# Tetramputechture/nclone

Measured on AMD Instinct MI355X. Metric: env-steps/sec (whole node) at N parallel envs, higher is better.
Workload: dtype f64

## Files before the change

include/npp_amd.h:

```cpp
#ifndef NPP_AMD_H
#define NPP_AMD_H

#include <stdint.h>

#ifdef __cplusplus
extern "C" {
#endif

typedef struct npp_handle_s *npp_handle;

enum {
    NPP_OK = 0,
    NPP_ERR_INVALID = 1,
    NPP_ERR_HIP = 2,
    NPP_ERR_UNSUPPORTED = 3,
    NPP_ERR_STATE = 4
};

enum {
    NPP_FLAG_AUTORESET = 1u << 0,
    NPP_FLAG_ALLOW_UNSUPPORTED = 1u << 1,
    NPP_FLAG_FRAME_CENTERED = 1u << 2,
    NPP_FLAG_FAST_RESET = 1u << 3
};
// ... 47 lines not shown
int npp_set_truncation_limit(npp_handle h, const int32_t *limits, int32_t all);
int npp_set_dynamic_truncation(npp_handle h, int enable);
int npp_level_truncation_limit(const double *map, int64_t n, int32_t *limit, int32_t *surface_area);

int npp_step(npp_handle h, const uint8_t *d_actions, int frame_skip, const npp_step_out *out);

int npp_step_many(npp_handle h, const uint8_t *d_actions, int n_steps, int frame_skip, const npp_step_out *out);

int npp_tick(npp_handle h, const uint8_t *d_inputs, int n_ticks);

int npp_observe(npp_handle h, const npp_step_out *out);

int npp_render_player_frame(npp_handle h, uint8_t *d_out);
int npp_set_entity_pos(npp_handle h, int env, int kind, double x, double y);

int npp_switch_states(npp_handle h, float *d_out);

int npp_reachability(npp_handle h, float *d_features, float *d_mine_sdf, int32_t *d_status);
int npp_reachability_ex(npp_handle h, float *d_features, float *d_mine_sdf, int32_t *d_status, float *d_switch_states);

int npp_set_minimal_observation(npp_handle h, int enable);
int npp_minimal_encode_host(const uint32_t *state_a, const double *planes, int count, float *out);
int npp_minimal_observation(npp_handle h, float *d_out , int32_t *d_status );

int npp_render_frame(npp_handle h, int env0, int count, uint8_t *d_out);

int npp_render_global_view(npp_handle h, uint8_t *d_out);

int npp_dump_state(npp_handle h, int env0, int count, double *f64_out, int32_t *i32_out);

int npp_dump_entities(npp_handle h, int env, int32_t *out, int max, int *n_out);

int npp_dump_level_segments(npp_handle h, int level, int16_t *out, int max_rows, int *n_out);

int npp_compile_level_segments(const double *map, int64_t n, int16_t *out, int max_rows, int *n_out,
                               uint32_t *unsupported_mask);
int npp_compile_level_entities(const double *map, int64_t n, double *out, int max_rows, int *n_out);

int npp_set_step_variant(npp_handle h, int variant);
int npp_get_step_variant(npp_handle h, int *variant, int *tuned);

int npp_set_obs_overlap(npp_handle h, int percent);
int npp_set_obs_overlap_parts(npp_handle h, const int *cuts, int n_cuts);
int npp_join(npp_handle h);

int npp_reach_compile(const double *map, int64_t n, int32_t *info, uint8_t *base_in, uint8_t *base_adj, uint8_t *phys, uint8_t *in,
// ... 43 lines not shown
```

nclone_amd/_native.py:

```python
import ctypes as C
import os

_HERE = os.path.dirname(os.path.abspath(__file__))
LIB_PATH = os.environ.get("NPP_AMD_LIB") or os.path.join(_HERE, "libnpp_amd.so")

NPP_OK = 0
NPP_ERR_INVALID, NPP_ERR_HIP, NPP_ERR_UNSUPPORTED, NPP_ERR_STATE = 1, 2, 3, 4
FLAG_AUTORESET = 1
FLAG_ALLOW_UNSUPPORTED = 2
FLAG_FRAME_CENTERED = 4
FLAG_FAST_RESET = 8
F_WON, F_DEAD, F_SWITCH, F_TRUNCATED, F_CAUSE_MINE, F_CAUSE_IMPACT = 1, 2, 4, 8, 16, 32
GAME_STATE_DIM = 41
MINIMAL_OBS_DIM = 40
DUMP_F64 = 12
DUMP_I32 = 32

EXPORTS = [
    "npp_create", "npp_destroy", "npp_last_error", "npp_set_stream", "npp_sync", "npp_load_levels",
    "npp_assign_levels", "npp_reset", "npp_set_truncation_limit", "npp_step", "npp_tick", "npp_observe",
    "npp_render_player_frame", "npp_dump_state", "npp_dump_entities", "npp_dump_level_segments",
    "npp_compile_level_segments", "npp_compile_level_entities", "npp_set_step_variant", "npp_get_step_variant", "npp_num_envs", "npp_num_levels",
    "npp_set_launch_geometry", "npp_get_launch_geometry", "npp_snapshot", "npp_restore", "npp_entity_checksum", "npp_compile_level_zoo", "npp_render_global_view", "npp_switch_states", "npp_set_entity_pos", "npp_step_many", "npp_render_frame", "npp_plan_zoo_block", "npp_reset_ex",
    "npp_reachability", "npp_reachability_ex", "npp_reach_compile", "npp_reach_features_host", "npp_reach_compile_miss", "npp_reach_rollout_host", "npp_set_dynamic_truncation", "npp_level_truncation_limit",
    "npp_set_obs_overlap", "npp_set_obs_overlap_parts", "npp_join",
    "npp_set_frame_stack", "npp_frame_stack_render", "npp_frame_stack_push", "npp_frame_stack_view",
    "npp_set_level_pool", "npp_draw_levels", "npp_get_env_levels", "npp_env_level_view", "npp_level_pool_draw_host",
    "npp_graph_observation", "npp_graph_compile",
    "npp_set_minimal_observation", "npp_minimal_observation", "npp_minimal_encode_host",
]


class StepOut(C.Structure):
    _fields_ = [
        ("d_game_state", C.c_void_p),
        ("d_action_mask", C.c_void_p),
        ("d_entity_pos", C.c_void_p),
        ("d_flags", C.c_void_p),
        ("d_reward", C.c_void_p),
        ("d_frames", C.c_void_p),
        ("d_terminal_state", C.c_void_p),
        ("d_spatial_context", C.c_void_p),
        ("d_positions", C.c_void_p),
        ("d_work", C.c_void_p),
    ]


class NativeLibraryMissing(RuntimeError):
    pass


_lib = None
# ... 55 lines not shown
    L.npp_reach_features_host.argtypes = [C.POINTER(C.c_double), C.c_int64, C.c_void_p, C.c_void_p, C.c_int, C.c_void_p, C.c_void_p,
                                          C.c_void_p]
    L.npp_reach_compile_miss.argtypes = [C.POINTER(C.c_double), C.c_int64] + [C.c_void_p] * 4
    L.npp_reach_rollout_host.argtypes = [C.POINTER(C.c_double), C.c_int64, C.c_void_p, C.c_void_p, C.c_void_p, C.c_int, C.c_void_p, C.c_void_p, C.c_void_p]
    L.npp_set_dynamic_truncation.argtypes = [H, C.c_int]
    L.npp_level_truncation_limit.argtypes = [C.POINTER(C.c_double), C.c_int64, C.POINTER(C.c_int32), C.POINTER(C.c_int32)]
    L.npp_snapshot.argtypes = [H]
    L.npp_restore.argtypes = [H, C.POINTER(C.c_uint8)]
    L.npp_set_frame_stack.argtypes = [H, C.c_int, C.c_int, C.c_int]
    L.npp_frame_stack_render.argtypes = [H]
    L.npp_frame_stack_push.argtypes = [H, C.c_void_p, C.c_void_p, C.c_void_p, C.c_int, C.c_int, C.c_void_p]
    L.npp_frame_stack_view.argtypes = [H, C.c_int, C.POINTER(C.c_void_p), C.POINTER(C.c_int64), C.POINTER(C.c_int64)]
    L.npp_set_level_pool.argtypes = [H, C.POINTER(C.c_double), C.c_int, C.c_uint64]
    L.npp_draw_levels.argtypes = [H, C.POINTER(C.c_uint8)]
    L.npp_get_env_levels.argtypes = [H, C.POINTER(C.c_int32)]
    L.npp_env_level_view.argtypes = [H, C.POINTER(C.c_void_p)]
    L.npp_graph_observation.argtypes = [H, C.c_void_p, C.c_void_p, C.c_void_p, C.c_void_p, C.c_int]
    L.npp_graph_compile.argtypes = [C.POINTER(C.c_double), C.c_int64, C.c_void_p, C.c_void_p, C.c_void_p]
    L.npp_level_pool_draw_host.argtypes = [C.POINTER(C.c_double), C.c_int, C.c_uint64, C.POINTER(C.c_int32), C.POINTER(C.c_uint32), C.c_int,
                                           C.POINTER(C.c_int32)]
    L.npp_set_minimal_observation.argtypes = [H, C.c_int]
    L.npp_minimal_observation.argtypes = [H, C.c_void_p, C.c_void_p]
    L.npp_minimal_encode_host.argtypes = [C.c_void_p, C.c_void_p, C.c_int, C.c_void_p]
    L.npp_num_envs.argtypes = [H]
    L.npp_num_levels.argtypes = [H]
    for name in EXPORTS:
        if name != "npp_last_error":
            getattr(L, name).restype = C.c_int
    _lib = L
    return L


class NppError(RuntimeError):
    def __init__(self, code, msg):
        super().__init__("npp error %d: %s" % (code, msg))
        self.code = code


def check(handle, code):
    if code != NPP_OK:
        msg = lib().npp_last_error(handle)
        raise NppError(code, msg.decode() if msg else "?")
```

nclone_amd/build_native.py:

```python
import os
import subprocess
import sys

HERE = os.path.dirname(os.path.abspath(__file__))
CSRC = os.path.join(HERE, "csrc")
OUT = os.path.join(HERE, "libnpp_amd.so")
SOURCES = ["npp_kernels.hip", "npp_render.hip", "npp_stack.hip", "npp_pool.hip", "npp_reach_kernel.hip", "npp_graph.hip", "npp_capi.cpp", "npp_level.cpp", "npp_reach.cpp",
           "npp_graph.cpp", "npp_host.cpp"]
HEADERS = ["npp_internal.hpp", "npp_level.hpp", "npp_zoo.hpp", "npp_reach.hpp", "npp_reach_build.hpp", "npp_reach_features.hpp",
           "npp_host.hpp", "npp_zoo_layout.hpp", "npp_pool.hpp", "npp_graph.hpp", "npp_minimal.hpp",
           "npp_reach_tables.inc", os.path.join("..", "..", "include", "npp_amd.h")]


def needs_build():
    if not os.path.isfile(OUT):
        return True
    t = os.path.getmtime(OUT)
    for f in SOURCES + HEADERS:
        if os.path.getmtime(os.path.join(CSRC, f)) > t:
            return True
    return False


def build(force=False, verbose=False, out=None, extra_flags=()):
    if out is None and not force and not needs_build():
        return OUT
    hipcc = os.environ.get("HIPCC", "/opt/rocm/bin/hipcc")
    objdir = os.path.join(HERE, "_obj") if out is None else out + "_obj"
    out = OUT if out is None else out
    os.makedirs(objdir, exist_ok=True)
    flags = ["--offload-arch=gfx950", "-O3", "-std=c++17", "-fPIC", "-ffp-contract=off", "-fno-fast-math", "-Wall",
             "-Wno-unused-function", "-Wno-unused-value", "-Wno-unused-result", "-I", os.path.join(HERE, "..", "include")]
    flags += list(extra_flags)
# ... 43 lines not shown
```

nclone_amd/csrc/npp_host.cpp:

```cpp
#include "npp_host.hpp"

#include <cstring>

#include "../../include/npp_amd.h"
#include "npp_minimal.hpp"
#include "npp_pool.hpp"
#include "npp_reach_build.hpp"

using namespace npp;

namespace npp {
std::string &host_error() {
    static thread_local std::string e;
    return e;
}
}

namespace {
int fail(std::nullptr_t, int code, const std::string &msg) {
    host_error() = msg;
    return code;
}
}

extern "C" {

int npp_minimal_encode_host(const uint32_t *state_a, const double *planes, int count, float *out) {
    if (count < 0 || (count > 0 && (!state_a || !planes || !out))) return fail(nullptr, NPP_ERR_INVALID, "npp_minimal_encode_host: bad arguments");
    for (int i = 0; i < count; i++)
        minobs_encode_state(state_a[i], planes[4 * i], planes[4 * i + 1], planes[4 * i + 2], planes[4 * i + 3], out + (size_t)i * MINOBS_DIM);
    return NPP_OK;
}

int npp_level_pool_draw_host(const double *weights, int n_levels, uint64_t seed, const int32_t *envs, const uint32_t *counts, int count,
                             int32_t *out) {
    if (count < 0 || (count > 0 && (!envs || !counts || !out))) return fail(nullptr, NPP_ERR_INVALID, "npp_level_pool_draw_host: bad arguments");
    std::vector<double> cdf;
    int last = 0;
    std::string err;
    if (!pool_cdf(weights, n_levels, n_levels, cdf, last, err)) return fail(nullptr, NPP_ERR_INVALID, err);
    for (int i = 0; i < count; i++) out[i] = pool_pick(cdf.data(), n_levels, last, seed, (uint32_t)envs[i], counts[i]);
    return NPP_OK;
}

int npp_compile_level_segments(const double *map, int64_t n, int16_t *out, int max_rows, int *n_out, uint32_t *unsupported_mask) {
    if (!map || !out || !n_out) return fail(nullptr, NPP_ERR_INVALID, "npp_compile_level_segments: bad arguments");
    CompiledLevel L;
    std::string err;
    if (!compile_level(map, n, L, err)) return fail(nullptr, NPP_ERR_INVALID, "npp_compile_level_segments: " + err);
    int r = dump_segments(L, out, max_rows);
    if (r < 0) return fail(nullptr, NPP_ERR_INVALID, "npp_compile_level_segments: buffer too small");
    *n_out = r;
    if (unsupported_mask) *unsupported_mask = L.unsupported_mask;
// ... 85 lines not shown
```

nclone_amd/csrc/npp_kernels.hip:

```cpp
#include <hip/hip_runtime.h>

#include <algorithm>
#include <vector>

#include <type_traits>

#include "npp_internal.hpp"
#include "npp_level.hpp"

#pragma clang fp contract(off)

namespace npp {
namespace {

constexpr double NINJA_RADIUS = 10.0;
constexpr double GRAVITY_FALL = 0.06666666666666665;
constexpr double GRAVITY_JUMP = 0.01111111111111111;
constexpr double GROUND_ACCEL = 0.06666666666666665;
constexpr double AIR_ACCEL = 0.04444444444444444;
constexpr double DRAG_REGULAR = 0.9933221725495059;
constexpr double DRAG_SLOW = 0.8617738760127536;
constexpr double FRICTION_GROUND = 0.9459290248857720;
constexpr double FRICTION_GROUND_SLOW = 0.8617738760127536;
constexpr double FRICTION_WALL = 0.9113380468927672;
constexpr double MAX_HOR_SPEED = 3.333;
constexpr int MAX_JUMP_DURATION = 45;
constexpr double MAX_SURVIVABLE_IMPACT = 6.0;
constexpr double TWO_THIRDS = 2.0 / 3;
constexpr double LEN45 = 0x1.0f876ccdf6cd9p+5;
// ... 461 lines not shown
    0x1.db00000000000p+9 ,
    0x1.e100000000000p+9 ,
    0x1.e700000000000p+9 ,
    0x1.ed00000000000p+9 ,
    0x1.f300000000000p+9 ,
    0x1.f900000000000p+9 ,
    0x1.fefffffffffffp+9 ,
    0x1.0280000000000p+10 ,
    0x1.0580000000000p+10
};

template <int K> struct Cand {
    double rx0, ry0, rx1, ry1;
    bool ok;
    uint32_t s[K];
    double x1[K], y1[K], x2[K], y2[K];
    double wx[K], wy[K], l2[K], rl2[K];
    double ox[K], oy[K];
    double bx0[K], by0[K], bx1[K], by1[K];
    double tx0[K], tx1[K], ty0[K], ty1[K];
};

template <int G, int K>
DEV void cand_gather(const Lv &lv, int r, double qx0, double qy0, double qx1, double qy1, Cand<K> &c) {
    const int c0x = cell_coord(qx0, 43), c1x = cell_coord(qx1, 43), c0y = cell_coord(qy0, 24), c1y = cell_coord(qy1, 24);
    c.rx0 = 24.0 * c0x; c.rx1 = 24.0 * (c1x + 1); c.ry0 = 24.0 * c0y; c.ry1 = 24.0 * (c1y + 1);
    const int ncol = c1x - c0x + 1;
    int a0 = lv.seg_start[c0x * 25 + c0y], n0 = lv.seg_start[c0x * 25 + c1y + 1] - a0;
    int a1 = 0, n1 = 0, a2 = 0, n2 = 0;
    if (ncol > 1) { a1 = lv.seg_start[(c0x + 1) * 25 + c0y]; n1 = lv.seg_start[(c0x + 1) * 25 + c1y + 1] - a1; }
    if (ncol > 2) { a2 = lv.seg_start[(c0x + 2) * 25 + c0y]; n2 = lv.seg_start[(c0x + 2) * 25 + c1y + 1] - a2; }
    const int total = n0 + n1 + n2;
    c.ok = ncol <= 3 && total <= G * K;
#pragma unroll
    for (int k = 0; k < K; k++) {
        int f = k * G + r;
        c.s[k] = 0;
        c.x1[k] = 0; c.y1[k] = 0; c.x2[k] = 0; c.y2[k] = 0; c.wx[k] = 0; c.wy[k] = 0; c.l2[k] = 1; c.rl2[k] = 1;
        c.ox[k] = 0; c.oy[k] = 0; c.bx0[k] = 0; c.by0[k] = 0; c.bx1[k] = 0; c.by1[k] = 0;
        c.tx0[k] = 0; c.tx1[k] = 0; c.ty0[k] = 0; c.ty1[k] = 0;
        if (c.ok && f < total) {
            int xc = c0x, i = a0 + f;
            if (f >= n0) { xc += 1; i = a1 + (f - n0); }
            if (f >= n0 + n1) { xc += 1; i = a2 + (f - n0 - n1); }
            uint32_t s = lv.segs[i];
            int yc = s >> 11;
            uint32_t cb = lv.bounds[xc * 25 + yc];
            c.s[k] = s | ((uint32_t)xc << 16) | 0x80000000u;
// ... 629 lines not shown
    if (in_jump_buffer || new_jump_check) {
        if (n.walled || in_wall_buffer) { wall_jump(n); return; }
        if (in_floor_buffer) { floor_jump(n); return; }
        if (lp && in_lp_buffer && new_jump_check) {
            n.fbuf = -1; n.wbuf = -1; n.jbuf = -1; n.lbuf = -1;
            double boost_scalar = 2 * dabs(lp[0]) + 2;
            if (boost_scalar == 2) boost_scalar = 1.7;
            n.vx += lp[0] * boost_scalar * TWO_THIRDS;
            n.vy += lp[1] * boost_scalar * TWO_THIRDS;
            return;
        }
    }
    if (!n.walled) {
        if (n.state == 5) n.state = 4;
    } else if (n.state == 5) {
        if (n.hor * n.wn <= 0) n.vy *= FRICTION_WALL;
        else n.state = 4;
    } else if (n.vy > 0 && n.hor * n.wn < 0) {
        if (n.state == 3) n.gjump = 0;
        n.state = 5;
    }
}

template <int G, bool ZOO, int V>
DEV void sim_tick(const Lv &lv, const Zoo &z, int r, Nj &n, EntBits eb, int hor, int jump, int n_ent STAMP_ARG) {
    constexpr int K = VariantK<G, ZOO, V>::value;
    STAMP_INIT;
    asm volatile("" : "+v"(hor), "+v"(jump));
    n.frame += 1;
    n.hor = hor;
    n.jump = jump;
    const bool zoo = ZOO && z.on;
    if (zoo) zoo_entities_tick<G>(lv, z, r, n, eb, n_ent);
    else think_mines(lv, n, eb);
    STAMP(2);
    if (n.state == 9) return;
    if (n.state != 6) {
        double drag = n.dslow ? DRAG_SLOW : DRAG_REGULAR;
        n.vx *= drag;
        n.vy *= drag;
        n.vy += n.gjump ? GRAVITY_JUMP : GRAVITY_FALL;
        double xold = n.x, yold = n.y;
        n.x += n.vx;
        n.y += n.vy;
        n.vxo = n.vx; n.vyo = n.vy;
        n.fcount = 0; n.ccount = 0;
        double fnsx = 0, fnsy = 0, cnsx = 0, cnsy = 0;
        ZTick zt;
        zt.xcr = 0; zt.ycr = 0; zt.clen = 0; zt.crushable = 0; zt.gcx = 0; zt.gcy = 0; zt.phys_near = false;
        if (zoo) zoo_pre_collision<G>(lv, z, r, n, zt);
        if constexpr (!ZOO) {
            if (r == 0) {
                double *sp = lv.spill;
                sp[0] = n.vxo; sp[1] = n.vyo; sp[2] = n.fnx; sp[3] = n.fny; sp[4] = n.cnx; sp[5] = n.cny;
                int *ip = reinterpret_cast<int *>(sp + 8);
                ip[0] = n.fair; ip[1] = n.scf; ip[2] = n.frame; ip[3] = n.gold; ip[4] = n.doors; ip[5] = n.fastord;
            }
            asm volatile("" ::: "memory");
        }
        Cand<K> cd;
        {
            const double pad = NINJA_RADIUS + 2.2;
            cand_gather<G, K>(lv, r, (xold < n.x ? xold : n.x) - pad, (yold < n.y ? yold : n.y) - pad,
                              (xold > n.x ? xold : n.x) + pad, (yold > n.y ? yold : n.y) + pad, cd);
        }
        STAMP(3);
        Crush cr{0, 0, 0};
        for (int k = 0; k < 4; k++) {
            const double xb = n.x, yb = n.y;
            if (zoo && zt.phys_near) {
                cr.xcr = zt.xcr; cr.ycr = zt.ycr; cr.clen = zt.clen;
                collide_vs_objects<G>(lv, z, r, n, zt, xold, yold, fnsx, fnsy, cnsx, cnsy);
                cr.xcr = zt.xcr; cr.ycr = zt.ycr; cr.clen = zt.clen;
            }
            const int applied = collide_vs_tiles<G, K, ZOO>(lv, r, n, cd, xold, yold, fnsx, fnsy, cnsx, cnsy, cr STAMP_PASS);
            n.work += applied;
            zt.xcr = cr.xcr; zt.ycr = cr.ycr; zt.clen = cr.clen;
            if (!(zoo && zt.phys_near) && applied == 0 && n.x == xb && n.y == yb) break;
        }
        STAMP(4);
        if constexpr (!ZOO) {
            asm volatile("" ::: "memory");
            const double *sp = lv.spill;
            n.vxo = sp[0]; n.vyo = sp[1]; n.fnx = sp[2]; n.fny = sp[3]; n.cnx = sp[4]; n.cny = sp[5];
            const int *ip = reinterpret_cast<const int *>(sp + 8);
            n.fair = ip[0]; n.scf = ip[1]; n.frame = ip[2]; n.gold = ip[3]; n.doors = ip[4]; n.fastord = ip[5];
        }
        post_collision<G, K, ZOO>(lv, z, r, n, cd, eb, fnsx, fnsy, cnsx, cnsy, xold, yold, zt);
        STAMP(5);
    }
    ninja_think(n, zoo ? z.blk : nullptr);
    STAMP(6);
}

DEV void write_game_state(const Nj &n, int limit, float *o ) {
    double vmag = dsqrt(sq(n.vx) + sq(n.vy));
    o[0] = (float)(pymin(vmag / (MAX_HOR_SPEED * 2), 1.0) * 2 - 1);
    bool mv = vmag > 1e-6;
    o[1] = (float)(mv ? n.vx / vmag : 0.0);
    o[2] = (float)(mv ? n.vy / vmag : 0.0);
    o[3] = (n.state <= 2) ? 1.f : -1.f;
    o[4] = (n.state == 3 || n.state == 4) ? 1.f : -1.f;
    o[5] = (n.state == 5) ? 1.f : -1.f;
    o[6] = (n.state >= 6 && n.state <= 9) ? 1.f : -1.f;
    o[7] = n.airborn ? 1.f : -1.f;
    o[8] = (float)n.hor;
    o[9] = n.jump ? 1.f : -1.f;
    o[10] = (float)(((n.jbuf > 0 ? n.jbuf : 0) / 5.0) * 2 - 1);
    o[11] = (float)(((n.fbuf > 0 ? n.fbuf : 0) / 5.0) * 2 - 1);
    o[12] = (float)(((n.wbuf > 0 ? n.wbuf : 0) / 5.0) * 2 - 1);
    o[13] = (float)((n.fcount < 1 ? n.fcount : 1) * 2 - 1);
    o[14] = -1.f;
    o[15] = (float)((n.ccount < 1 ? n.ccount : 1) * 2 - 1);
    o[16] = (float)(dsqrt(sq(n.fnx) + sq(n.fny)) * 2 - 1);
    o[17] = 0.f;
    o[18] = (float)n.fny;
    double g = n.gjump ? GRAVITY_JUMP : GRAVITY_FALL;
    o[19] = (float)((g - GRAVITY_JUMP) / (GRAVITY_FALL - GRAVITY_JUMP) * 2 - 1);
    o[20] = n.walled ? 1.f : -1.f;
    o[21] = (float)n.fnx;
    o[22] = (float)n.cnx;
    o[23] = (float)n.cny;
    double drag = n.dslow ? DRAG_SLOW : DRAG_REGULAR;
    o[24] = (float)((drag - DRAG_SLOW) / (DRAG_REGULAR - DRAG_SLOW) * 2 - 1);
    o[25] = (float)((FRICTION_GROUND - FRICTION_GROUND_SLOW) / (FRICTION_GROUND - FRICTION_GROUND_SLOW) * 2 - 1);
    o[26] = (float)pymax(-1.0, pymin(1.0, (n.vx - n.vxo) / MAX_HOR_SPEED));
    o[27] = (float)pymax(-1.0, pymin(1.0, (n.vy - n.vyo) / MAX_HOR_SPEED));
    o[28] = (float)(pymin(vmag / (MAX_HOR_SPEED * 1.5), 1.0) * 2 - 1);
    o[29] = (float)(pymin(n.fair / 60.0, 1.0) * 2 - 1);
    o[30] = (float)(pymin(n.jdur / (double)MAX_JUMP_DURATION, 1.0) * 2 - 1);
    o[31] = (float)(pymin(n.scf / 30.0, 1.0) * 2 - 1);
    double ke = 0.5 * (sq(n.vx) + sq(n.vy));
    o[32] = (float)(pymin(ke / sq(MAX_HOR_SPEED), 1.0) * 2 - 1);
    o[33] = (float)((n.y / 600.0) * 2 - 1);
    double fm = dsqrt(sq(g) + sq(!n.airborn ? GROUND_ACCEL : AIR_ACCEL));
    o[34] = (float)(pymin(fm / 0.1, 1.0) * 2 - 1);
    double pke = 0.5 * (sq(n.vxo) + sq(n.vyo));
    o[35] = (float)pymax(-1.0, pymin(1.0, (ke - pke) / pymax(ke + 0.01, 0.01)));
    o[36] = (float)(pymin(n.fcount / 5.0, 1.0) * 2 - 1);
    o[37] = -1.f;
    o[38] = (float)(atan2(n.fny, n.fnx) / 3.141592653589793);
    o[39] = n.walled ? (float)n.wn : 0.f;
    o[40] = (float)(limit <= 0 ? 1.0 : pymax(0.0, (double)(limit - n.frame) / (double)limit));
}

DEV uint32_t action_mask_bits(const Nj &n) {
    uint32_t mask = 0x3f;
    bool has_active_buffer = (-1 < n.jbuf && n.jbuf < 5) || (-1 < n.fbuf && n.fbuf < 5) || (-1 < n.wbuf && n.wbuf < 5) ||
                             (-1 < n.lbuf && n.lbuf < 4);
    if (n.airborn && n.state != 3 && n.jump != 0 && !has_active_buffer) mask &= ~(8u | 16u | 32u);
    if (n.walled) {
        bool masks_dir = !n.airborn || n.state == 5 || !(n.vy >= 0);
        if (masks_dir) { if (n.wn > 0) mask &= ~2u; else if (n.wn < 0) mask &= ~4u; }
    }
    if (!mask) mask = 1;
    return mask;
}

template <int G>
DEV void write_spatial_context(const KernelArgs &a, const LevelHdr &H, Nj &n, EntBits eb, int env, int r, bool valid) {
    if (!valid) return;
    float *out = a.out.spatial_context + (size_t)env * 112;
    float *cache = a.sc_cache + (size_t)env * 48;
    const uint8_t *tiles = a.blob + H.off_tiles;
    const int col = floor12(n.x) >> 1, row = floor12(n.y) >> 1;
    for (int k = r; k < 64; k += G) {
        int rr = row - 4 + (k >> 3), cc = col - 4 + (k & 7);
// ... 98 lines not shown
    spawn_state(lv, n);
    n.fastord = episode;
    if (fast) {
        n.fastord |= 1;
        lv.perm = reinterpret_cast<const uint16_t *>(a.blob + H.off_ent_perm);
        const uint32_t *keep = reinterpret_cast<const uint32_t *>(a.blob + H.off_keep_words);
        for (int w = 0; w < nw; w++) {
            const uint32_t k = keep[w];
            eb.w[w * eb.stride] = (eb.w[w * eb.stride] & k) | (lv.init_words[w] & ~k);
        }
        if constexpr (ZOO) {
            z.ent_ord = reinterpret_cast<const uint16_t *>(a.blob + H.off_ent_rank);
            if (z.on) zoo_fast_reset_block(z, r, G);
        }
    } else {
        lv.perm = reinterpret_cast<const uint16_t *>(a.blob + H.off_ent_ident);
        for (int w = 0; w < nw; w++) eb.w[w * eb.stride] = lv.init_words[w];
        if constexpr (ZOO) {
            z.ent_ord = z.ent_seq;
            if (z.on) zoo_init_block(z, r, G, false);
        }
    }
}

template <int G, bool LDS_LEVEL, bool ZOO, bool MANY, int V>
DEV void run(const KernelArgs &a, unsigned char *smem) {
    constexpr int EPW = WAVE / G;
    const int tid = threadIdx.x;
    const int wave = tid >> 6;
    const int lane = tid & 63;
    const int r = lane & (G - 1);
    const int epb = EPW * (blockDim.x >> 6);
    const int eib = wave * EPW + lane / G;
    const int blk = a.wg_order ? (int)a.wg_order[blockIdx.x + a.wg_first] : (int)blockIdx.x + a.wg_first;
    const unsigned long long wg_t0 = a.wg_cost ? __builtin_amdgcn_s_memtime() : 0ull;
    const int env0 = blk * epb;
    const int env = env0 + eib;
    const bool in_range = env < a.n;
    const bool valid = in_range && (!a.obs_mask || a.obs_mask[env] != 0);
    if (a.obs_mask && !__syncthreads_or(valid)) return;
    const int e = in_range ? env : a.n - 1;
    const int n_valid = (a.n - env0) < epb ? (a.n - env0) : epb;

    uint32_t *ew = reinterpret_cast<uint32_t *>(smem + (LDS_LEVEL ? a.lds_hot_cap : 0u));
    uint32_t *stage = ew + (size_t)a.n_words_max * epb;
    EntBits eb;
// ... 67 lines not shown
#ifdef NPP_STAMPS
    Stamps st;
    for (int i = 0; i < N_STAMP; i++) st.acc[i] = 0;
#endif
    STAMP_INIT;
    Nj n;
    load_state(a, e, n);
    lv.perm = reinterpret_cast<const uint16_t *>(a.blob + ((n.fastord & 1) ? H.off_ent_perm : H.off_ent_ident));
    if constexpr (ZOO) {
        if (n.fastord & 1) z.ent_ord = reinterpret_cast<const uint16_t *>(a.blob + H.off_ent_rank);
    }
    const int nw = (int)lv.n_words;
    if (r == 0)
        for (int w = 0; w < nw; w++) eb.w[w * eb.stride] = a.ent_bits[(size_t)w * a.n + e];
    __syncthreads();

    STAMP(0);
    uint32_t flags = 0;
    int executed = 0;
    float reward = 0.f;
    bool done = false;
    const bool stepping = a.mode == 0 && a.n_ticks > 0;
    const bool writer = valid && r == 0;
    const int n_steps = MANY ? (a.n_steps > 1 ? a.n_steps : 1) : 1;
#pragma nounroll
    for (int sidx = 0; sidx < n_steps; sidx++) {
        flags = 0; executed = 0; reward = 0.f;
        n.work = 0;
        const bool had_switch = lv.obs_switch >= 0 && ent_get(eb, lv.obs_switch) == 0;
        {
            const bool gym = a.mode == 0;
            const int act = (gym && a.n_ticks > 0) ? a.inputs[(size_t)sidx * a.n + e] : 0;
            int hor = (act == 1 || act == 4) ? -1 : ((act == 2 || act == 5) ? 1 : 0);
            int jump = act >= 3 ? 1 : 0;
            bool live = valid && !(gym && (n.state == 8 || n.state == 6 || n.state == 7));
            for (int t = 0; t < a.n_ticks; t++) {
                if (!gym) {
                    const int b = a.inputs[(size_t)t * a.n + e];
                    const int l = (b >> 2) & 1, rr = (b >> 1) & 1;
                    hor = (l && rr) ? 0 : (l ? -1 : (rr ? 1 : 0));
                    jump = b & 1;
                }
                if (live) {
                    sim_tick<G, ZOO, V>(lv, z, r, n, eb, hor, jump, (int)H.n_ent STAMP_PASS);
                    executed++;
                    if (gym && (n.state == 8 || n.state == 6 || n.state == 7)) live = false;
                }
                if (!__any(live)) break;
            }
        }

        STAMP(1);
        const bool sw_now = lv.obs_switch >= 0 ? ent_get(eb, lv.obs_switch) == 0 : true;
        if (n.state == 8) flags |= 1u;
        if (n.state == 6 || n.state == 7) flags |= 2u;
        if (sw_now) flags |= 4u;
        if (n.cause == 1) flags |= 16u;
        if (n.cause == 2) flags |= 32u;
        done = (flags & 3u) != 0;
        if (stepping && !done && n.frame >= a.trunc_limit[e]) { flags |= 8u; done = true; }
        if (flags & 1u) reward += 20.f;
        if (flags & 2u) reward -= 3.f;
        if (sw_now && !had_switch && lv.obs_switch >= 0) reward += 10.f;

        if (writer) {
            const size_t o = (size_t)sidx * a.n + env;
            if (a.out.flags) a.out.flags[o] = (uint8_t)flags;
            if (a.out.reward) a.out.reward[o] = reward;
            if (a.out.frames) a.out.frames[o] = (uint16_t)executed;
            if (a.out.work) a.out.work[o] = (uint16_t)(n.work > 0xffff ? 0xffff : n.work);
        }
        if (MANY && sidx + 1 < n_steps && a.autoreset && stepping && done)
            episode_reset<ZOO>(a, H, lv, z, n, eb, nw, r, G);
    }

    const bool do_reset = a.autoreset && stepping && done;
#pragma nounroll
    for (int pass = (a.out.terminal_state ? 0 : 1); pass < 2; pass++) {
        if (pass == 1 && do_reset) episode_reset<ZOO>(a, H, lv, z, n, eb, nw, r, G);
        float *gdst = pass == 0 ? a.out.terminal_state : a.out.game_state;
        if (gdst) {
            if (r == 0) write_game_state(n, a.trunc_limit[e], reinterpret_cast<float *>(stage) + eib * 41);
            __syncthreads();
            if (pass == 1 && !a.obs_mask) {
                block_store_rows(stage, reinterpret_cast<uint32_t *>(gdst + (size_t)env0 * 41), 41, n_valid);
            } else if ((pass == 1 || do_reset) && writer) {
                const uint32_t *row = stage + eib * 41;
                uint32_t *dst = reinterpret_cast<uint32_t *>(gdst + (size_t)env * 41);
                for (int k = 0; k < 41; k++) dst[k] = row[k];
            }
            __syncthreads();
        }
    }
    if (a.out.entity_pos) {
        if (r == 0) {
            float *row = reinterpret_cast<float *>(stage) + eib * 6;
            row[0] = (float)(n.x / 1056.0); row[1] = (float)(n.y / 600.0);
            row[2] = (float)((ZOO ? lv.sw_x : H.sw_x) / 1056.0); row[3] = (float)((ZOO ? lv.sw_y : H.sw_y) / 600.0);
            row[4] = (float)((ZOO ? lv.door_x : H.door_x) / 1056.0); row[5] = (float)((ZOO ? lv.door_y : H.door_y) / 600.0);
        }
        __syncthreads();
        if (!a.obs_mask) {
            block_store_rows(stage, reinterpret_cast<uint32_t *>(a.out.entity_pos + (size_t)env0 * 6), 6, n_valid);
        } else if (writer) {
            const uint32_t *row = stage + eib * 6;
            uint32_t *dst = reinterpret_cast<uint32_t *>(a.out.entity_pos + (size_t)env * 6);
            for (int k = 0; k < 6; k++) dst[k] = row[k];
        }
        __syncthreads();
    }
    if (a.out.positions && writer) {
        double *row = a.out.positions + (size_t)env * 6;
        row[0] = n.x; row[1] = n.y;
        row[2] = ZOO ? lv.sw_x : H.sw_x; row[3] = ZOO ? lv.sw_y : H.sw_y; row[4] = ZOO ? lv.door_x : H.door_x; row[5] = ZOO ? lv.door_y : H.door_y;
    }
    if (a.out.spatial_context) write_spatial_context<G>(a, H, n, eb, env, r, valid);
    if (a.out.action_mask && writer) {
        uint32_t m = action_mask_bits(n);
        int8_t *row = a.out.action_mask + (size_t)env * 6;
        for (int k = 0; k < 6; k++) row[k] = (int8_t)((m >> k) & 1u);
    }

    STAMP(7);
    if (writer) {
        store_state(a, env, n);
        for (int w = 0; w < nw; w++) a.ent_bits[(size_t)w * a.n + env] = eb.w[w * eb.stride];
    }
    if constexpr (ZOO) {
        if (valid && z.on) {
            const int used = ZOO_HEAD + z.door_words + ZOO_MOV_WORDS * z.n_mov;
            double *dst = a.zoo + (size_t)env * a.zoo_words;
            for (int k = r; k < used; k += G) dst[k] = z.blk[k];
        }
    }
    STAMP(8);
    if (a.wg_cost && lane == 0) atomicMax(&a.wg_cost[blk], (uint32_t)(__builtin_amdgcn_s_memtime() - wg_t0));
#ifdef NPP_STAMPS
    if (lane == 0) {
        unsigned gw = blockIdx.x * (blockDim.x >> 6) + wave;
        if (gw < 16384)
            for (int i = 0; i < N_STAMP; i++) g_stamps[gw * N_STAMP + i] += st.acc[i];
    }
#endif
}

template <int G, bool LDS_LEVEL, bool ZOO, bool MANY, int V>
__global__ __launch_bounds__(256, (ZOO ? 1 : ((G < 16 || V == 2) ? 1 : 2))) void npp_step_kernel(KernelArgs a) {
    extern __shared__ __align__(16) unsigned char smem[];
    run<G, LDS_LEVEL, ZOO, MANY, V>(a, smem);
}
// ... 175 lines not shown
```

Baseline: 91.49 million.

## Cache collision candidates across ticks, hand off epilogue to one wave, table-driven game state

```diff
diff --git a/include/npp_amd.h b/include/npp_amd.h
--- a/include/npp_amd.h
+++ b/include/npp_amd.h
@@ -93,6 +93,7 @@
 int npp_set_minimal_observation(npp_handle h, int enable);
 int npp_minimal_encode_host(const uint32_t *state_a, const double *planes, int count, float *out);
 int npp_minimal_observation(npp_handle h, float *d_out , int32_t *d_status );
+int npp_game_state_encode_host(const double *f64, const int32_t *i32, const int32_t *limit, int count, float *out);
 
 int npp_render_frame(npp_handle h, int env0, int count, uint8_t *d_out);
 
diff --git a/nclone_amd/_native.py b/nclone_amd/_native.py
--- a/nclone_amd/_native.py
+++ b/nclone_amd/_native.py
@@ -28,6 +28,7 @@
     "npp_set_level_pool", "npp_draw_levels", "npp_get_env_levels", "npp_env_level_view", "npp_level_pool_draw_host",
     "npp_graph_observation", "npp_graph_compile",
     "npp_set_minimal_observation", "npp_minimal_observation", "npp_minimal_encode_host",
+    "npp_game_state_encode_host",
 ]
 
 
@@ -129,6 +130,7 @@
     L.npp_set_minimal_observation.argtypes = [H, C.c_int]
     L.npp_minimal_observation.argtypes = [H, C.c_void_p, C.c_void_p]
     L.npp_minimal_encode_host.argtypes = [C.c_void_p, C.c_void_p, C.c_int, C.c_void_p]
+    L.npp_game_state_encode_host.argtypes = [C.c_void_p, C.c_void_p, C.c_void_p, C.c_int, C.c_void_p]
     L.npp_num_envs.argtypes = [H]
     L.npp_num_levels.argtypes = [H]
     for name in EXPORTS:
diff --git a/nclone_amd/build_native.py b/nclone_amd/build_native.py
--- a/nclone_amd/build_native.py
+++ b/nclone_amd/build_native.py
@@ -8,7 +8,7 @@
 SOURCES = ["npp_kernels.hip", "npp_render.hip", "npp_stack.hip", "npp_pool.hip", "npp_reach_kernel.hip", "npp_graph.hip", "npp_capi.cpp", "npp_level.cpp", "npp_reach.cpp",
            "npp_graph.cpp", "npp_host.cpp"]
 HEADERS = ["npp_internal.hpp", "npp_level.hpp", "npp_zoo.hpp", "npp_reach.hpp", "npp_reach_build.hpp", "npp_reach_features.hpp",
-           "npp_host.hpp", "npp_zoo_layout.hpp", "npp_pool.hpp", "npp_graph.hpp", "npp_minimal.hpp",
+           "npp_host.hpp", "npp_zoo_layout.hpp", "npp_pool.hpp", "npp_graph.hpp", "npp_minimal.hpp", "npp_game_state.hpp",
            "npp_reach_tables.inc", os.path.join("..", "..", "include", "npp_amd.h")]
 
 
diff --git a/nclone_amd/csrc/npp_game_state.hpp b/nclone_amd/csrc/npp_game_state.hpp
--- /dev/null
+++ b/nclone_amd/csrc/npp_game_state.hpp
@@ -0,0 +1,121 @@
+#pragma once
+#include <cmath>
+#include <cstdint>
+
+#if defined(__HIPCC__) || defined(__HIP__)
+#define NPP_GS_HD __host__ __device__ inline __attribute__((always_inline))
+#else
+#define NPP_GS_HD inline
+#endif
+
+namespace npp {
+namespace gs {
+
+constexpr int DIM = 41;
+constexpr double GRAVITY_FALL = 0.06666666666666665;
+constexpr double GRAVITY_JUMP = 0.01111111111111111;
+constexpr double GROUND_ACCEL = 0.06666666666666665;
+constexpr double AIR_ACCEL = 0.04444444444444444;
+constexpr double DRAG_REGULAR = 0.9933221725495059;
+constexpr double DRAG_SLOW = 0.8617738760127536;
+constexpr double FRICTION_GROUND = 0.9459290248857720;
+constexpr double FRICTION_GROUND_SLOW = 0.8617738760127536;
+constexpr double MAX_HOR_SPEED = 3.333;
+constexpr int MAX_JUMP_DURATION = 45;
+
+constexpr double pmin(double a, double b) { return b < a ? b : a; }
+constexpr double pmax(double a, double b) { return b > a ? b : a; }
+constexpr int clampi(int v, int lo, int hi) { return v < lo ? lo : (v > hi ? hi : v); }
+
+constexpr float f_buffer(int b) { return (float)(((b > 0 ? b : 0) / 5.0) * 2 - 1); }
+constexpr float f_fair(int v) { return (float)(pmin(v / 60.0, 1.0) * 2 - 1); }
+constexpr float f_jdur(int v) { return (float)(pmin(v / (double)MAX_JUMP_DURATION, 1.0) * 2 - 1); }
+constexpr float f_scf(int v) { return (float)(pmin(v / 30.0, 1.0) * 2 - 1); }
+constexpr float f_fcount5(int v) { return (float)(pmin(v / 5.0, 1.0) * 2 - 1); }
+constexpr float f_count1(int v) { return (float)((v < 1 ? v : 1) * 2 - 1); }
+constexpr float f_gravity(bool gjump) {
+    return (float)(((gjump ? GRAVITY_JUMP : GRAVITY_FALL) - GRAVITY_JUMP) / (GRAVITY_FALL - GRAVITY_JUMP) * 2 - 1);
+}
+constexpr float f_drag(bool dslow) {
+    return (float)(((dslow ? DRAG_SLOW : DRAG_REGULAR) - DRAG_SLOW) / (DRAG_REGULAR - DRAG_SLOW) * 2 - 1);
+}
+constexpr float F_FRICTION =
+    (float)((FRICTION_GROUND - FRICTION_GROUND_SLOW) / (FRICTION_GROUND - FRICTION_GROUND_SLOW) * 2 - 1);
+
+constexpr int N_BUF = 8, N_FAIR = 61, N_JDUR = MAX_JUMP_DURATION + 1, N_SCF = 31, N_FCOUNT5 = 6, N_COUNT1 = 2;
+template <int N> struct Tab { float v[N]; };
+template <int N, float (*F)(int)> constexpr Tab<N> make_tab() {
+    Tab<N> t{};
+    for (int i = 0; i < N; i++) t.v[i] = F(i);
+    return t;
+}
+
+struct State {
+    double y, vx, vy, vxo, vyo, fnx, fny, cnx, cny;
+    int state, airborn, walled, wn, hor, jump, gjump, dslow;
+    int jbuf, fbuf, wbuf, fcount, ccount, fair, jdur, scf, frame;
+};
+constexpr int STATE_F64 = 9, STATE_I32 = 17;
+
+template <class N>
+NPP_GS_HD void write_game_state(const N &n, int limit, float *o ) {
+    static constexpr Tab<N_BUF> T_BUF = make_tab<N_BUF, f_buffer>();
+    static constexpr Tab<N_FAIR> T_FAIR = make_tab<N_FAIR, f_fair>();
+    static constexpr Tab<N_JDUR> T_JDUR = make_tab<N_JDUR, f_jdur>();
+    static constexpr Tab<N_SCF> T_SCF = make_tab<N_SCF, f_scf>();
+    static constexpr Tab<N_FCOUNT5> T_FCOUNT5 = make_tab<N_FCOUNT5, f_fcount5>();
+    static constexpr Tab<N_COUNT1> T_COUNT1 = make_tab<N_COUNT1, f_count1>();
+    const double vx = n.vx, vy = n.vy, vxo = n.vxo, vyo = n.vyo, fnx = n.fnx, fny = n.fny;
+    const int state = (int)n.state;
+    const bool airborn = n.airborn != 0, walled = n.walled != 0, gjump = n.gjump != 0;
+    double vmag = __builtin_sqrt(vx * vx + vy * vy);
+    o[0] = (float)(pmin(vmag / (MAX_HOR_SPEED * 2), 1.0) * 2 - 1);
+    bool mv = vmag > 1e-6;
+    o[1] = (float)(mv ? vx / vmag : 0.0);
+    o[2] = (float)(mv ? vy / vmag : 0.0);
+    o[3] = (state <= 2) ? 1.f : -1.f;
+    o[4] = (state == 3 || state == 4) ? 1.f : -1.f;
+    o[5] = (state == 5) ? 1.f : -1.f;
+    o[6] = (state >= 6 && state <= 9) ? 1.f : -1.f;
+    o[7] = airborn ? 1.f : -1.f;
+    o[8] = (float)(int)n.hor;
+    o[9] = n.jump ? 1.f : -1.f;
+    o[10] = T_BUF.v[clampi((int)n.jbuf, 0, N_BUF - 1)];
+    o[11] = T_BUF.v[clampi((int)n.fbuf, 0, N_BUF - 1)];
+    o[12] = T_BUF.v[clampi((int)n.wbuf, 0, N_BUF - 1)];
+    o[13] = T_COUNT1.v[clampi((int)n.fcount, 0, N_COUNT1 - 1)];
+    o[14] = -1.f;
+    o[15] = T_COUNT1.v[clampi((int)n.ccount, 0, N_COUNT1 - 1)];
+    o[16] = (float)(__builtin_sqrt(fnx * fnx + fny * fny) * 2 - 1);
+    o[17] = 0.f;
+    o[18] = (float)fny;
+    o[19] = gjump ? f_gravity(true) : f_gravity(false);
+    o[20] = walled ? 1.f : -1.f;
+    o[21] = (float)fnx;
+    o[22] = (float)n.cnx;
+    o[23] = (float)n.cny;
+    o[24] = n.dslow ? f_drag(true) : f_drag(false);
+    o[25] = F_FRICTION;
+    o[26] = (float)pmax(-1.0, pmin(1.0, (vx - vxo) / MAX_HOR_SPEED));
+    o[27] = (float)pmax(-1.0, pmin(1.0, (vy - vyo) / MAX_HOR_SPEED));
+    o[28] = (float)(pmin(vmag / (MAX_HOR_SPEED * 1.5), 1.0) * 2 - 1);
+    o[29] = T_FAIR.v[clampi((int)n.fair, 0, N_FAIR - 1)];
+    o[30] = T_JDUR.v[clampi((int)n.jdur, 0, N_JDUR - 1)];
+    o[31] = T_SCF.v[clampi((int)n.scf, 0, N_SCF - 1)];
+    double ke = 0.5 * (vx * vx + vy * vy);
+    o[32] = (float)(pmin(ke / (MAX_HOR_SPEED * MAX_HOR_SPEED), 1.0) * 2 - 1);
+    o[33] = (float)((n.y / 600.0) * 2 - 1);
+    const double g = gjump ? GRAVITY_JUMP : GRAVITY_FALL;
+    double fm = __builtin_sqrt(g * g + (!airborn ? GROUND_ACCEL * GROUND_ACCEL : AIR_ACCEL * AIR_ACCEL));
+    o[34] = (float)(pmin(fm / 0.1, 1.0) * 2 - 1);
+    double pke = 0.5 * (vxo * vxo + vyo * vyo);
+    o[35] = (float)pmax(-1.0, pmin(1.0, (ke - pke) / pmax(ke + 0.01, 0.01)));
+    o[36] = T_FCOUNT5.v[clampi((int)n.fcount, 0, N_FCOUNT5 - 1)];
+    o[37] = -1.f;
+    o[38] = (float)(atan2(fny, fnx) / 3.141592653589793);
+    o[39] = walled ? (float)(int)n.wn : 0.f;
+    o[40] = (float)(limit <= 0 ? 1.0 : pmax(0.0, (double)(limit - (int)n.frame) / (double)limit));
+}
+
+}
+}
diff --git a/nclone_amd/csrc/npp_host.cpp b/nclone_amd/csrc/npp_host.cpp
--- a/nclone_amd/csrc/npp_host.cpp
+++ b/nclone_amd/csrc/npp_host.cpp
@@ -3,6 +3,7 @@
 #include <cstring>
 
 #include "../../include/npp_amd.h"
+#include "npp_game_state.hpp"
 #include "npp_minimal.hpp"
 #include "npp_pool.hpp"
 #include "npp_reach_build.hpp"
@@ -29,6 +30,21 @@
     if (count < 0 || (count > 0 && (!state_a || !planes || !out))) return fail(nullptr, NPP_ERR_INVALID, "npp_minimal_encode_host: bad arguments");
     for (int i = 0; i < count; i++)
         minobs_encode_state(state_a[i], planes[4 * i], planes[4 * i + 1], planes[4 * i + 2], planes[4 * i + 3], out + (size_t)i * MINOBS_DIM);
+    return NPP_OK;
+}
+
+int npp_game_state_encode_host(const double *f64, const int32_t *i32, const int32_t *limit, int count, float *out) {
+    if (count < 0 || (count > 0 && (!f64 || !i32 || !limit || !out))) return fail(nullptr, NPP_ERR_INVALID, "npp_game_state_encode_host: bad arguments");
+    for (int i = 0; i < count; i++) {
+        const double *f = f64 + (size_t)i * gs::STATE_F64;
+        const int32_t *k = i32 + (size_t)i * gs::STATE_I32;
+        gs::State n;
+        n.y = f[0]; n.vx = f[1]; n.vy = f[2]; n.vxo = f[3]; n.vyo = f[4]; n.fnx = f[5]; n.fny = f[6]; n.cnx = f[7]; n.cny = f[8];
+        n.state = k[0]; n.airborn = k[1]; n.walled = k[2]; n.wn = k[3]; n.hor = k[4]; n.jump = k[5]; n.gjump = k[6]; n.dslow = k[7];
+        n.jbuf = k[8]; n.fbuf = k[9]; n.wbuf = k[10]; n.fcount = k[11]; n.ccount = k[12]; n.fair = k[13]; n.jdur = k[14]; n.scf = k[15];
+        n.frame = k[16];
+        gs::write_game_state(n, limit[i], out + (size_t)i * gs::DIM);
+    }
     return NPP_OK;
 }
 
diff --git a/nclone_amd/csrc/npp_kernels.hip b/nclone_amd/csrc/npp_kernels.hip
--- a/nclone_amd/csrc/npp_kernels.hip
+++ b/nclone_amd/csrc/npp_kernels.hip
@@ -5,6 +5,7 @@
 
 #include <type_traits>
 
+#include "npp_game_state.hpp"
 #include "npp_internal.hpp"
 #include "npp_level.hpp"
 
@@ -512,8 +513,7 @@
 };
 
 template <int G, int K>
-DEV void cand_gather(const Lv &lv, int r, double qx0, double qy0, double qx1, double qy1, Cand<K> &c) {
-    const int c0x = cell_coord(qx0, 43), c1x = cell_coord(qx1, 43), c0y = cell_coord(qy0, 24), c1y = cell_coord(qy1, 24);
+DEV void cand_gather(const Lv &lv, int r, int c0x, int c1x, int c0y, int c1y, Cand<K> &c) {
     c.rx0 = 24.0 * c0x; c.rx1 = 24.0 * (c1x + 1); c.ry0 = 24.0 * c0y; c.ry1 = 24.0 * (c1y + 1);
     const int ncol = c1x - c0x + 1;
     int a0 = lv.seg_start[c0x * 25 + c0y], n0 = lv.seg_start[c0x * 25 + c1y + 1] - a0;
@@ -1189,8 +1189,9 @@
     }
 }
 
-template <int G, bool ZOO, int V>
-DEV void sim_tick(const Lv &lv, const Zoo &z, int r, Nj &n, EntBits eb, int hor, int jump, int n_ent STAMP_ARG) {
+template <int G, bool ZOO, int V, bool KEEP>
+DEV void sim_tick(const Lv &lv, const Zoo &z, int r, Nj &n, EntBits eb, int hor, int jump, int n_ent,
+                  Cand<VariantK<G, ZOO, V>::value> &kept, int &kept_range STAMP_ARG) {
     constexpr int K = VariantK<G, ZOO, V>::value;
     STAMP_INIT;
     asm volatile("" : "+v"(hor), "+v"(jump));
@@ -1225,11 +1226,17 @@
             }
             asm volatile("" ::: "memory");
         }
-        Cand<K> cd;
+        Cand<K> local;
+        Cand<K> &cd = KEEP ? kept : local;
         {
             const double pad = NINJA_RADIUS + 2.2;
-            cand_gather<G, K>(lv, r, (xold < n.x ? xold : n.x) - pad, (yold < n.y ? yold : n.y) - pad,
-                              (xold > n.x ? xold : n.x) + pad, (yold > n.y ? yold : n.y) + pad, cd);
+            const int c0x = cell_coord((xold < n.x ? xold : n.x) - pad, 43), c1x = cell_coord((xold > n.x ? xold : n.x) + pad, 43);
+            const int c0y = cell_coord((yold < n.y ? yold : n.y) - pad, 24), c1y = cell_coord((yold > n.y ? yold : n.y) + pad, 24);
+            const int range = c0x | (c1x << 6) | (c0y << 12) | (c1y << 18);
+            if (!KEEP || __any(range != kept_range)) {
+                cand_gather<G, K>(lv, r, c0x, c1x, c0y, c1y, cd);
+                kept_range = range;
+            }
         }
         STAMP(3);
         Crush cr{0, 0, 0};
@@ -1260,56 +1267,12 @@
     STAMP(6);
 }
 
-DEV void write_game_state(const Nj &n, int limit, float *o ) {
-    double vmag = dsqrt(sq(n.vx) + sq(n.vy));
-    o[0] = (float)(pymin(vmag / (MAX_HOR_SPEED * 2), 1.0) * 2 - 1);
-    bool mv = vmag > 1e-6;
-    o[1] = (float)(mv ? n.vx / vmag : 0.0);
-    o[2] = (float)(mv ? n.vy / vmag : 0.0);
-    o[3] = (n.state <= 2) ? 1.f : -1.f;
-    o[4] = (n.state == 3 || n.state == 4) ? 1.f : -1.f;
-    o[5] = (n.state == 5) ? 1.f : -1.f;
-    o[6] = (n.state >= 6 && n.state <= 9) ? 1.f : -1.f;
-    o[7] = n.airborn ? 1.f : -1.f;
-    o[8] = (float)n.hor;
-    o[9] = n.jump ? 1.f : -1.f;
-    o[10] = (float)(((n.jbuf > 0 ? n.jbuf : 0) / 5.0) * 2 - 1);
-    o[11] = (float)(((n.fbuf > 0 ? n.fbuf : 0) / 5.0) * 2 - 1);
-    o[12] = (float)(((n.wbuf > 0 ? n.wbuf : 0) / 5.0) * 2 - 1);
-    o[13] = (float)((n.fcount < 1 ? n.fcount : 1) * 2 - 1);
-    o[14] = -1.f;
-    o[15] = (float)((n.ccount < 1 ? n.ccount : 1) * 2 - 1);
-    o[16] = (float)(dsqrt(sq(n.fnx) + sq(n.fny)) * 2 - 1);
-    o[17] = 0.f;
-    o[18] = (float)n.fny;
-    double g = n.gjump ? GRAVITY_JUMP : GRAVITY_FALL;
-    o[19] = (float)((g - GRAVITY_JUMP) / (GRAVITY_FALL - GRAVITY_JUMP) * 2 - 1);
-    o[20] = n.walled ? 1.f : -1.f;
-    o[21] = (float)n.fnx;
-    o[22] = (float)n.cnx;
-    o[23] = (float)n.cny;
-    double drag = n.dslow ? DRAG_SLOW : DRAG_REGULAR;
-    o[24] = (float)((drag - DRAG_SLOW) / (DRAG_REGULAR - DRAG_SLOW) * 2 - 1);
-    o[25] = (float)((FRICTION_GROUND - FRICTION_GROUND_SLOW) / (FRICTION_GROUND - FRICTION_GROUND_SLOW) * 2 - 1);
-    o[26] = (float)pymax(-1.0, pymin(1.0, (n.vx - n.vxo) / MAX_HOR_SPEED));
-    o[27] = (float)pymax(-1.0, pymin(1.0, (n.vy - n.vyo) / MAX_HOR_SPEED));
-    o[28] = (float)(pymin(vmag / (MAX_HOR_SPEED * 1.5), 1.0) * 2 - 1);
-    o[29] = (float)(pymin(n.fair / 60.0, 1.0) * 2 - 1);
-    o[30] = (float)(pymin(n.jdur / (double)MAX_JUMP_DURATION, 1.0) * 2 - 1);
-    o[31] = (float)(pymin(n.scf / 30.0, 1.0) * 2 - 1);
-    double ke = 0.5 * (sq(n.vx) + sq(n.vy));
-    o[32] = (float)(pymin(ke / sq(MAX_HOR_SPEED), 1.0) * 2 - 1);
-    o[33] = (float)((n.y / 600.0) * 2 - 1);
-    double fm = dsqrt(sq(g) + sq(!n.airborn ? GROUND_ACCEL : AIR_ACCEL));
-    o[34] = (float)(pymin(fm / 0.1, 1.0) * 2 - 1);
-    double pke = 0.5 * (sq(n.vxo) + sq(n.vyo));
-    o[35] = (float)pymax(-1.0, pymin(1.0, (ke - pke) / pymax(ke + 0.01, 0.01)));
-    o[36] = (float)(pymin(n.fcount / 5.0, 1.0) * 2 - 1);
-    o[37] = -1.f;
-    o[38] = (float)(atan2(n.fny, n.fnx) / 3.141592653589793);
-    o[39] = n.walled ? (float)n.wn : 0.f;
-    o[40] = (float)(limit <= 0 ? 1.0 : pymax(0.0, (double)(limit - n.frame) / (double)limit));
-}
+using gs::write_game_state;
+static_assert(gs::GRAVITY_FALL == GRAVITY_FALL && gs::GRAVITY_JUMP == GRAVITY_JUMP && gs::GROUND_ACCEL == GROUND_ACCEL &&
+              gs::AIR_ACCEL == AIR_ACCEL && gs::DRAG_REGULAR == DRAG_REGULAR && gs::DRAG_SLOW == DRAG_SLOW &&
+              gs::FRICTION_GROUND == FRICTION_GROUND && gs::FRICTION_GROUND_SLOW == FRICTION_GROUND_SLOW &&
+              gs::MAX_HOR_SPEED == MAX_HOR_SPEED && gs::MAX_JUMP_DURATION == MAX_JUMP_DURATION,
+              "npp_game_state.hpp keeps other physics constants than the step kernels");
 
 DEV uint32_t action_mask_bits(const Nj &n) {
     uint32_t mask = 0x3f;
@@ -1454,6 +1417,17 @@
         }
     }
 }
+
+struct EpiRow {
+    Nj n;
+    uint32_t meta;
+    float reward;
+    int work;
+    int pad_;
+    double sw_x, sw_y, door_x, door_y;
+};
+static_assert(sizeof(Nj) == 128 && alignof(EpiRow) == 8 && sizeof(EpiRow) == 176 && sizeof(EpiRow) <= LDS_SPILL_BYTES &&
+              LDS_SPILL_BYTES % 8 == 0, "the epilogue hand-off row must fit the 8-byte aligned LDS spill row");
 
 template <int G, bool LDS_LEVEL, bool ZOO, bool MANY, int V>
 DEV void run(const KernelArgs &a, unsigned char *smem) {
@@ -1567,7 +1541,10 @@
     bool done = false;
     const bool stepping = a.mode == 0 && a.n_ticks > 0;
     const bool writer = valid && r == 0;
+    const bool handoff = epb <= WAVE;
     const int n_steps = MANY ? (a.n_steps > 1 ? a.n_steps : 1) : 1;
+    Cand<VariantK<G, ZOO, V>::value> kept;
+    int kept_range = -1;
 #pragma nounroll
     for (int sidx = 0; sidx < n_steps; sidx++) {
         flags = 0; executed = 0; reward = 0.f;
@@ -1587,7 +1564,7 @@
                     jump = b & 1;
                 }
                 if (live) {
-                    sim_tick<G, ZOO, V>(lv, z, r, n, eb, hor, jump, (int)H.n_ent STAMP_PASS);
+                    sim_tick<G, ZOO, V, !ZOO && !MANY>(lv, z, r, n, eb, hor, jump, (int)H.n_ent, kept, kept_range STAMP_PASS);
                     executed++;
                     if (gym && (n.state == 8 || n.state == 6 || n.state == 7)) live = false;
                 }
@@ -1608,24 +1585,49 @@
         if (flags & 2u) reward -= 3.f;
         if (sw_now && !had_switch && lv.obs_switch >= 0) reward += 10.f;
 
-        if (writer) {
+        if (writer && !(handoff && sidx + 1 == n_steps)) {
             const size_t o = (size_t)sidx * a.n + env;
             if (a.out.flags) a.out.flags[o] = (uint8_t)flags;
             if (a.out.reward) a.out.reward[o] = reward;
             if (a.out.frames) a.out.frames[o] = (uint16_t)executed;
             if (a.out.work) a.out.work[o] = (uint16_t)(n.work > 0xffff ? 0xffff : n.work);
         }
-        if (MANY && sidx + 1 < n_steps && a.autoreset && stepping && done)
+        if (MANY && sidx + 1 < n_steps && a.autoreset && stepping && done) {
             episode_reset<ZOO>(a, H, lv, z, n, eb, nw, r, G);
+        }
     }
 
     const bool do_reset = a.autoreset && stepping && done;
+    EpiRow *const myrow = reinterpret_cast<EpiRow *>(lv.spill);
+    const EpiRow *const xrow = reinterpret_cast<const EpiRow *>(lv.spill - (size_t)eib * (LDS_SPILL_BYTES / 8)) + (handoff ? lane : eib);
+    const bool epi = handoff ? (wave == 0 && lane < n_valid) : (r == 0);
+    const int xeib = handoff ? lane : eib;
+    const int xenv = env0 + xeib;
+    const int xe = handoff ? (epi ? xenv : e) : e;
+    if (handoff && r == 0) {
+        myrow->meta = (flags & 0xffu) | ((uint32_t)(executed & 0xffff) << 8) | (valid ? 1u << 24 : 0u);
+        myrow->reward = reward;
+        myrow->work = n.work;
+        if (a.out.entity_pos || a.out.positions) {
+            myrow->sw_x = ZOO ? lv.sw_x : H.sw_x; myrow->sw_y = ZOO ? lv.sw_y : H.sw_y;
+            myrow->door_x = ZOO ? lv.door_x : H.door_x; myrow->door_y = ZOO ? lv.door_y : H.door_y;
+        }
+    }
+    Nj m = n;
 #pragma nounroll
     for (int pass = (a.out.terminal_state ? 0 : 1); pass < 2; pass++) {
         if (pass == 1 && do_reset) episode_reset<ZOO>(a, H, lv, z, n, eb, nw, r, G);
+        if (handoff && pass == 1 && a.out.spatial_context) write_spatial_context<G>(a, H, n, eb, env, r, valid);
         float *gdst = pass == 0 ? a.out.terminal_state : a.out.game_state;
+        if (handoff) {
+            if (r == 0) myrow->n = n;
+            __syncthreads();
+            if (epi) m = xrow->n;
+        } else {
+            m = n;
+        }
         if (gdst) {
-            if (r == 0) write_game_state(n, a.trunc_limit[e], reinterpret_cast<float *>(stage) + eib * 41);
+            if (epi) write_game_state(m, a.trunc_limit[xe], reinterpret_cast<float *>(stage) + xeib * 41);
             __syncthreads();
             if (pass == 1 && !a.obs_mask) {
                 block_store_rows(stage, reinterpret_cast<uint32_t *>(gdst + (size_t)env0 * 41), 41, n_valid);
@@ -1637,12 +1639,18 @@
             __syncthreads();
         }
     }
+    const bool xvalid = handoff ? (epi && ((xrow->meta >> 24) & 1u)) : valid;
+    double sw_x = 0, sw_y = 0, door_x = 0, door_y = 0;
+    if ((a.out.entity_pos || a.out.positions) && epi) {
+        if (handoff) { sw_x = xrow->sw_x; sw_y = xrow->sw_y; door_x = xrow->door_x; door_y = xrow->door_y; }
+        else { sw_x = ZOO ? lv.sw_x : H.sw_x; sw_y = ZOO ? lv.sw_y : H.sw_y; door_x = ZOO ? lv.door_x : H.door_x; door_y = ZOO ? lv.door_y : H.door_y; }
+    }
     if (a.out.entity_pos) {
-        if (r == 0) {
-            float *row = reinterpret_cast<float *>(stage) + eib * 6;
-            row[0] = (float)(n.x / 1056.0); row[1] = (float)(n.y / 600.0);
-            row[2] = (float)((ZOO ? lv.sw_x : H.sw_x) / 1056.0); row[3] = (float)((ZOO ? lv.sw_y : H.sw_y) / 600.0);
-            row[4] = (float)((ZOO ? lv.door_x : H.door_x) / 1056.0); row[5] = (float)((ZOO ? lv.door_y : H.door_y) / 600.0);
+        if (epi) {
+            float *row = reinterpret_cast<float *>(stage) + xeib * 6;
+            row[0] = (float)(m.x / 1056.0); row[1] = (float)(m.y / 600.0);
+            row[2] = (float)(sw_x / 1056.0); row[3] = (float)(sw_y / 600.0);
+            row[4] = (float)(door_x / 1056.0); row[5] = (float)(door_y / 600.0);
         }
         __syncthreads();
         if (!a.obs_mask) {
@@ -1654,23 +1662,36 @@
         }
         __syncthreads();
     }
-    if (a.out.positions && writer) {
-        double *row = a.out.positions + (size_t)env * 6;
-        row[0] = n.x; row[1] = n.y;
-        row[2] = ZOO ? lv.sw_x : H.sw_x; row[3] = ZOO ? lv.sw_y : H.sw_y; row[4] = ZOO ? lv.door_x : H.door_x; row[5] = ZOO ? lv.door_y : H.door_y;
-    }
-    if (a.out.spatial_context) write_spatial_context<G>(a, H, n, eb, env, r, valid);
-    if (a.out.action_mask && writer) {
-        uint32_t m = action_mask_bits(n);
-        int8_t *row = a.out.action_mask + (size_t)env * 6;
-        for (int k = 0; k < 6; k++) row[k] = (int8_t)((m >> k) & 1u);
+    if (a.out.positions && epi && xvalid) {
+        double *row = a.out.positions + (size_t)xenv * 6;
+        row[0] = m.x; row[1] = m.y;
+        row[2] = sw_x; row[3] = sw_y; row[4] = door_x; row[5] = door_y;
+    }
+    if (!handoff && a.out.spatial_context) {
+        write_spatial_context<G>(a, H, n, eb, env, r, valid);
+        m.scvalid = n.scvalid;
+    }
+    if (a.out.action_mask && epi && xvalid) {
+        uint32_t mb = action_mask_bits(m);
+        int8_t *row = a.out.action_mask + (size_t)xenv * 6;
+        for (int k = 0; k < 6; k++) row[k] = (int8_t)((mb >> k) & 1u);
     }
 
     STAMP(7);
-    if (writer) {
-        store_state(a, env, n);
+    if (epi && xvalid) {
+        store_state(a, xenv, m);
+        if (handoff) {
+            const uint32_t meta = xrow->meta;
+            const int work = xrow->work;
+            const size_t o = (size_t)(n_steps - 1) * a.n + xenv;
+            if (a.out.flags) a.out.flags[o] = (uint8_t)(meta & 0xffu);
+            if (a.out.reward) a.out.reward[o] = xrow->reward;
+            if (a.out.frames) a.out.frames[o] = (uint16_t)((meta >> 8) & 0xffffu);
+            if (a.out.work) a.out.work[o] = (uint16_t)(work > 0xffff ? 0xffff : work);
+        }
+    }
+    if (writer)
         for (int w = 0; w < nw; w++) a.ent_bits[(size_t)w * a.n + env] = eb.w[w * eb.stride];
-    }
     if constexpr (ZOO) {
         if (valid && z.on) {
             const int used = ZOO_HEAD + z.door_words + ZOO_MOV_WORDS * z.n_mov;
```

Result: slower. 28.62 million (-68.7%).
